# jack-nie/bitcoin-miner

Hardware: AMD Instinct MI355X
Metric: GH/s (SHA-256 nonce search) at 1/2/4/8 MI355X; % of VALU int roofline (higher is better)
Workload: dtype u32

## Files before the change

### bitcoin-miner_amd/csrc/minehip.cpp

```cpp
#include <hip/hip_runtime.h>
#include <stdio.h>
#include <stdlib.h>
#include <string.h>

#include <algorithm>
#include <atomic>
#include <chrono>
#include <cmath>
#include <condition_variable>
#include <memory>
#include <mutex>
#include <string>
#include <system_error>
#include <thread>
#include <vector>

#include "../../include/minehip.h"
#include "../../include/minehip_server.h"
#include "layout.hpp"
#include "msgcodec.hpp"
#include "multi.hpp"
#include "plan.hpp"
#include "sched.hpp"

namespace mh {
hipError_t fast_module_init(int dev);
#ifdef MH_DEV_HOOKS
hipError_t fast_keep_ok(int dev, bool* ok);
hipError_t set_hash_xor(int dev, uint64_t x, hipStream_t s, bool* fast_ok);
#endif
hipError_t launch_fast(int dev, int J, int mode, const FastArgs& a, Partial* partials, hipStream_t s);
hipError_t launch_generic_scan(const GenArgs& a, Partial* partials, uint32_t blocks, hipStream_t s);
hipError_t launch_hash_batch(const GenArgs& a, const uint64_t* d_nonces, uint64_t* d_out, uint64_t n,
                             hipStream_t s);
hipError_t launch_merge(const Partial* partials, uint32_t n, Partial* best, hipStream_t s);
hipError_t launch_fast_first(int dev, int J, int mode, const FastArgs& a, Partial* partials, const FirstArgs& f,
                             bool stop, hipStream_t s);
hipError_t launch_generic_scan_first(const GenArgs& a, Partial* partials, uint32_t blocks, const FirstArgs& f,
                                     hipStream_t s);
hipError_t launch_finish_first(const GenArgs& a, const Partial* best, const unsigned long long* scanned, uint64_t* out,
                               hipStream_t s);
hipError_t launch_fast_hits(int dev, int J, int mode, const FastArgs& a, Partial* partials, const HitsArgs& h,
                            hipStream_t s);
hipError_t launch_generic_scan_hits(const GenArgs& a, Partial* partials, uint32_t blocks, const HitsArgs& h,
                                    hipStream_t s);
hipError_t launch_fast_hits_stop(int dev, int J, int mode, const FastArgs& a, Partial* partials, const HitsStopArgs& h,
                                 hipStream_t s);
hipError_t launch_generic_scan_hits_stop(const GenArgs& a, Partial* partials, uint32_t blocks, const HitsStopArgs& h,
                                         hipStream_t s);
hipError_t launch_batch_scan(const BatchEntry* entries, const uint32_t* tile_entry, Partial* partials, uint32_t tiles,
                             hipStream_t s);
hipError_t launch_merge_segments(const Partial* partials, const uint32_t* seg, Partial* results, uint32_t requests,
                                 hipStream_t s);
hipError_t launch_batch_scan_slots(const BatchEntry* entries, const uint32_t* tile_entry, Partial* partials,
                                   uint32_t tiles, hipStream_t s);
hipError_t launch_batch_fast(int dev, int J, int mode, const BatchFastItem* items, const uint32_t* chunk_item,
                             Partial* partials, uint32_t chunks, hipStream_t s);
#ifdef MH_DEV_HOOKS
hipError_t batch_fast_hooks(int dev, uint64_t x, hipStream_t s, bool* keep_ok, bool* xor_ok);
#endif
hipError_t launch_batch_scan_first(const BatchEntry* entries, const uint32_t* tile_entry, const uint32_t* entry_req,
                                   const uint32_t* order, BatchFirstWords* words, Partial* partials, uint32_t tiles,
                                   hipStream_t s);
hipError_t launch_merge_segments_first(const Partial* partials, const uint32_t* seg, const BatchEntry* entries,
                                       const uint32_t* tile_entry, const BatchFirstWords* words,
                                       BatchFirstResult* results, uint32_t requests, hipStream_t s);
hipError_t launch_batch_scan_first_slots(const BatchEntry* entries, const uint32_t* tile_entry,
                                         const uint32_t* entry_req, const uint32_t* order, BatchFirstWords* words,
                                         Partial* partials, uint32_t tiles, hipStream_t s);
hipError_t launch_merge_segments_first_ex(const Partial* partials, const uint32_t* seg, const GenArgs* req_gen,
                                          const BatchFirstWords* words, BatchFirstResult* results, uint32_t requests,
                                          hipStream_t s);
hipError_t launch_batch_first(int dev, int J, int mode, const BatchFirstItem* items, const uint32_t* chunk_item,
                              const uint32_t* order, Partial* partials, uint32_t chunks, hipStream_t s);
hipError_t launch_batch_stop(int dev, int J, int mode, const BatchFirstItem* items, const uint32_t* chunk_item,
                             const uint32_t* order, Partial* partials, uint32_t chunks, hipStream_t s);
hipError_t launch_batch_scan_hits(const BatchEntry* entries, const uint32_t* tile_entry, const uint32_t* entry_req,
                                  BatchHitsWords* words, Hit* hits, Partial* partials, uint32_t tiles,
                                  hipStream_t s);
hipError_t launch_batch_scan_hits_slots(const BatchEntry* entries, const uint32_t* tile_entry, const uint32_t* entry_req,
                                        BatchHitsWords* words, Hit* hits, Partial* partials, uint32_t tiles,
                                        hipStream_t s);
hipError_t launch_batch_hits(int dev, int J, int mode, const BatchHitsItem* items, const uint32_t* chunk_item,
                             Partial* partials, uint32_t chunks, hipStream_t s);
hipError_t launch_batch_scan_bound(bool slots, const BatchEntry* entries, const uint32_t* tile_entry,
                                   const uint32_t* entry_req, const uint32_t* order, BatchBoundWords* words,
                                   uint32_t* slices, Hit* hits, Partial* partials, uint32_t tiles, hipStream_t s);
hipError_t launch_batch_bound(int dev, int J, int mode, const BatchBoundItem* items, const uint32_t* chunk_item,
                              const uint32_t* order, Partial* partials, uint32_t chunks, hipStream_t s);
hipError_t launch_merge_segments_bound(const Partial* partials, const uint32_t* seg, const BatchBoundWords* words,
                                       const Hit* hits, Hit* packed, uint64_t limit, const unsigned long long* base_in,
                                       unsigned long long* base_out, BatchBoundResult* results, uint32_t requests,
                                       hipStream_t s);
hipError_t launch_merge_segments_hits(const Partial* partials, const uint32_t* seg, const BatchHitsWords* words,
                                      const Hit* hits, Hit* packed, uint64_t limit, const unsigned long long* base_in,
                                      unsigned long long* base_out, BatchHitsResult* results, uint32_t requests,
                                      hipStream_t s);
}

namespace {

using mh::Partial;

thread_local std::string g_err;

int fail(int code, const std::string& what) {
    g_err = what;
    return code;
}

}

namespace mh {
int set_error(int code, const char* what) { return fail(code, what); }
}

namespace {

#define MH_HIP(call)                                                                                 \
    do {                                                                                             \
        hipError_t e_ = (call);                                                                      \
        if (e_ != hipSuccess) return fail(MH_EHIP, std::string(#call) + ": " + hipGetErrorString(e_)); \
    } while (0)

constexpr uint64_t kBatchChunk = 1u << 22;
constexpr int kEventPairs = 512;
constexpr uint32_t kQueueSlots = 4096;
constexpr size_t kBatchTableBytes = 4u << 20;
constexpr uint32_t kBatchResults = 1u << 16;
constexpr size_t kFirstBatchFastTableBytes = 5u << 20;
static_assert(8u * (size_t)mh::kMaxBlocksPerLaunch + mh::kBatchMaxEntries * (sizeof(mh::BatchEntry) + 4u) +
                      (mh::kBatchMaxRequests + 1u) * 4u +
                      mh::kBatchMaxRequests * (sizeof(mh::GenArgs) + sizeof(mh::BatchFirstWords)) +
                      mh::kBatchMaxFastItems * sizeof(mh::BatchFirstItem) + 9u * 16u <= kFirstBatchFastTableBytes,
              "a first-hit pass with fast pieces fits its table buffer");
static_assert(8u * (size_t)mh::kMaxBlocksPerLaunch + mh::kBatchMaxEntries * (sizeof(mh::BatchEntry) + 4u) +
                      (mh::kBatchMaxRequests + 1u) * 4u + mh::kBatchMaxRequests * sizeof(mh::BatchBoundWords) +
                      mh::kBatchMaxFastItems * sizeof(mh::BatchBoundItem) + 9u * 16u <= kFirstBatchFastTableBytes,
              "a first-k-hits pass fits its table buffer");

struct Timed {
    hipEvent_t start = nullptr, stop = nullptr;
    int kind;
    int var;
};

struct VarStat {
    uint64_t launches = 0, nonces = 0, ns = 0, ops = 0, slots = 0;
};
constexpr int kVariants = 16 * mh::kModes * 5;
inline int var_index(int J, int mode, int L) { return J + 16 * mode + 16 * mh::kModes * (L - 1); }

struct DevCtx {
    std::mutex mu;
    int dev = -1;
    bool ready = false;
    hipStream_t stream = nullptr;
    hipStream_t ps[2] = {nullptr, nullptr};
    hipEvent_t ev_piece[2] = {nullptr, nullptr};
    hipEvent_t ev_main = nullptr;
    Partial* d_partials = nullptr;
    Partial* d_best = nullptr;
    Partial* h_best = nullptr;
    uint64_t* d_nonces = nullptr;
    uint64_t* d_hashes = nullptr;
    uint32_t poff = 0;
    uint32_t* d_counters = nullptr;
    uint32_t qoff = 0;
    uint8_t* d_btab = nullptr;
    uint8_t* h_btab = nullptr;
    Partial* d_bres = nullptr;
    Partial* h_bres = nullptr;
    mh::BatchFirstResult* d_fres = nullptr;
    mh::BatchFirstResult* h_fres = nullptr;
    uint8_t* d_ftab = nullptr;
    uint8_t* h_ftab = nullptr;
    uint64_t* d_first = nullptr;
    uint64_t* h_first = nullptr;
    const mh::FirstArgs* first = nullptr;
    bool first_stop = false;
    mh::Hit* d_hits = nullptr;
    uint64_t* d_hcursor = nullptr;
    uint64_t* h_hcursor = nullptr;
    const mh::HitsArgs* hits = nullptr;
    uint64_t* d_fhits = nullptr;
    uint32_t* d_slices = nullptr;
    uint64_t* h_fhits = nullptr;
    const mh::HitsStopArgs* hits_stop = nullptr;
    mh::BatchHitsResult* d_hres = nullptr;
    mh::BatchHitsResult* h_hres = nullptr;
    mh::Hit* d_hpacked = nullptr;
    uint64_t* d_hbase = nullptr;
    mh::BatchBoundResult* d_kres = nullptr;
    mh::BatchBoundResult* h_kres = nullptr;
    uint32_t* d_bslices = nullptr;
#ifdef MH_DEV_HOOKS
    uint32_t keep = 0;
    bool keep_fast = false;
    bool xor_on = false;
    bool xor_fast = false;
#endif
    bool prof = false;
    std::vector<Timed> pool;
    int used = 0;
    uint64_t cnt[8] = {0};
    VarStat var[kVariants];
};

std::mutex g_tab_mu;
std::vector<std::unique_ptr<DevCtx>> g_tab;
int g_ndev = -1;

int device_count_impl() {
    std::lock_guard<std::mutex> lk(g_tab_mu);
    if (g_ndev < 0) {
        int n = 0;
        if (hipGetDeviceCount(&n) != hipSuccess) n = 0;
        g_ndev = n;
        g_tab.resize((size_t)n);
        for (auto& p : g_tab) p.reset(new DevCtx());
    }
    return g_ndev;
}

int get_ctx(int dev, DevCtx** out) {
    const int n = device_count_impl();
    if (n <= 0) return fail(MH_ENODEV, "no HIP device visible");
    if (dev < 0 || dev >= n) return fail(MH_EINVAL, "device index out of range");
    DevCtx* c = g_tab[(size_t)dev].get();
    *out = c;
    return MH_OK;
}

int init_locked(DevCtx* c, int dev) {
    if (c->ready) return MH_OK;
    MH_HIP(hipSetDevice(dev));
    hipDeviceProp_t prop;
    MH_HIP(hipGetDeviceProperties(&prop, dev));
    if (strncmp(prop.gcnArchName, "gfx950", 6) != 0)
        return fail(MH_ENODEV, std::string("device is ") + prop.gcnArchName + ", kernels are built for gfx950 only");
    if (!c->stream) MH_HIP(hipStreamCreateWithFlags(&c->stream, hipStreamNonBlocking));
    if (!c->ps[0] || !c->ps[1]) {
        int least = 0, greatest = 0;
        MH_HIP(hipDeviceGetStreamPriorityRange(&least, &greatest));
        if (!c->ps[0]) MH_HIP(hipStreamCreateWithPriority(&c->ps[0], hipStreamNonBlocking, greatest));
        if (!c->ps[1]) MH_HIP(hipStreamCreateWithPriority(&c->ps[1], hipStreamNonBlocking, least));
    }
    for (auto& e : c->ev_piece)
        if (!e) MH_HIP(hipEventCreateWithFlags(&e, hipEventDisableTiming));
    if (!c->ev_main) MH_HIP(hipEventCreateWithFlags(&c->ev_main, hipEventDisableTiming));
    if (!c->d_partials) MH_HIP(hipMalloc(&c->d_partials, sizeof(Partial) * mh::kMaxBlocksPerLaunch));
    if (!c->d_best) MH_HIP(hipMalloc(&c->d_best, sizeof(Partial)));
    if (!c->d_counters) MH_HIP(hipMalloc(&c->d_counters, sizeof(uint32_t) * kQueueSlots));
    if (!c->h_best) MH_HIP(hipHostMalloc(&c->h_best, sizeof(Partial), hipHostMallocDefault));
    if (!c->d_nonces) MH_HIP(hipMalloc(&c->d_nonces, sizeof(uint64_t) * kBatchChunk));
    if (!c->d_hashes) MH_HIP(hipMalloc(&c->d_hashes, sizeof(uint64_t) * kBatchChunk));
    if (c->pool.empty()) c->pool.resize(kEventPairs);
    for (auto& t : c->pool) {
        if (!t.start) MH_HIP(hipEventCreate(&t.start));
        if (!t.stop) MH_HIP(hipEventCreate(&t.stop));
    }
    MH_HIP(mh::fast_module_init(dev));
    c->dev = dev;
    c->ready = true;
    return MH_OK;
}

#ifdef MH_DEV_HOOKS
int read_hash_keep(DevCtx* c) {
    c->keep = 0;
    c->keep_fast = false;
    const char* e = getenv("MINEHIP_DEV_HASH_KEEP");
    if (!e || !*e) return MH_OK;
    unsigned k0 = 0, k1 = 0;
    char rest = 0;
    if (sscanf(e, "%u,%u%c", &k0, &k1, &rest) != 2 || k0 > 32u || k1 > 32u)
        return fail(MH_EINVAL, "MINEHIP_DEV_HASH_KEEP: expected k0,k1 with 0 <= k <= 32");
    MH_HIP(mh::fast_keep_ok(c->dev, &c->keep_fast));
    c->keep = mh::keep_word(k0, k1);
    return MH_OK;
}

int read_hash_xor(DevCtx* c) {
    c->xor_on = c->xor_fast = false;
    const char* e = getenv("MINEHIP_DEV_HASH_XOR");
    uint64_t x = 0;
    if (e && *e) {
        size_t n = 0;
        for (; e[n]; ++n) {
            const char ch = e[n];
            const int v = (ch >= '0' && ch <= '9') ? ch - '0' : (ch >= 'a' && ch <= 'f') ? ch - 'a' + 10
                        : (ch >= 'A' && ch <= 'F') ? ch - 'A' + 10 : -1;
            if (v < 0 || n >= 16) return fail(MH_EINVAL, "MINEHIP_DEV_HASH_XOR: expected 1 to 16 hex digits");
            x = (x << 4) | (uint64_t)v;
        }
    }
    MH_HIP(mh::set_hash_xor(c->dev, x, c->stream, &c->xor_fast));
    c->xor_on = x != 0;
    return MH_OK;
}
#endif

int harvest_locked(DevCtx* c) {
    for (int i = 0; i < c->used; ++i) {
        float ms = 0.f;
        MH_HIP(hipEventElapsedTime(&ms, c->pool[(size_t)i].start, c->pool[(size_t)i].stop));
        const uint64_t ns = (uint64_t)((double)ms * 1.0e6);
        c->cnt[c->pool[(size_t)i].kind == 0 ? 2 : 5] += ns;
        if (c->pool[(size_t)i].kind == 0) c->var[c->pool[(size_t)i].var].ns += ns;
    }
    c->used = 0;
    return MH_OK;
}

int piece_streams_wait_main(DevCtx* c) {
    MH_HIP(hipEventRecord(c->ev_main, c->stream));
    for (auto s : c->ps) MH_HIP(hipStreamWaitEvent(s, c->ev_main, 0));
    return MH_OK;
}

int flush_partials(DevCtx* c, bool split) {
    if (!c->poff) return MH_OK;
    if (split) {
        for (int k = 0; k < 2; ++k) {
            MH_HIP(hipEventRecord(c->ev_piece[k], c->ps[k]));
            MH_HIP(hipStreamWaitEvent(c->stream, c->ev_piece[k], 0));
        }
    }
    MH_HIP(mh::launch_merge(c->d_partials, c->poff, c->d_best, c->stream));
    c->poff = 0;
    if (split) return piece_streams_wait_main(c);
    return MH_OK;
}

bool coarse_piece(const mh::Piece& p, const mh::PlanOpts& opt) { return p.kind == 0 && p.L == opt.lower_digits; }

bool early_piece_ok(const mh::FastArgs& a, int word) {
    const uint32_t J = (uint32_t)word;
    if ((a.inner >> 2) != J || a.hole + a.hole_w > a.n_hi + a.L) return false;
    for (uint32_t j = 0; j + 1u < a.L; ++j) {
        const uint32_t pos = a.g_last - j - (j >= a.g_hole ? 1u : 0u);
        if (pos > a.g_last || (pos >> 2) != J) return false;
    }
    return true;
}

int enqueue_piece(DevCtx* c, const mh::Piece& p, const mh::PlanOpts& opt, bool split) {
    hipStream_t s = !split ? c->stream : c->ps[coarse_piece(p, opt) ? 0 : 1];
    uint32_t blocks;
    if (p.kind == 0) {
        if (p.fa.n_runs == 0 || p.fa.L < 1 || p.fa.L > 5 || p.fa.n_hi + p.fa.L > 20)
            return fail(MH_EINTERNAL, "internal: bad fast piece");
        if (p.fa.mode >= mh::kModeOneEarly && !early_piece_ok(p.fa, p.J))
            return fail(MH_EINTERNAL, "internal: bad Early piece (an enumerated digit outside word J)");
        blocks = (p.fa.n_runs + mh::kBlockThreads - 1) / mh::kBlockThreads;
    } else {
        if (p.ga.count == 0 || p.ga.count > (uint64_t)mh::kMaxBlocksPerLaunch * mh::kBlockThreads)
            return fail(MH_EINTERNAL, "internal: bad generic piece");
        blocks = (uint32_t)((p.ga.count + mh::kBlockThreads - 1) / mh::kBlockThreads);
    }
    if (blocks > mh::kMaxBlocksPerLaunch) return fail(MH_EINTERNAL, "internal: grid too large");
    if (c->poff + blocks > mh::kMaxBlocksPerLaunch) {
        const int rc = flush_partials(c, split);
        if (rc) return rc;
    }
    Partial* out = c->d_partials + c->poff;
    Timed* tm = nullptr;
    mh::FastArgs fa = p.fa;
#ifdef MH_DEV_HOOKS
    mh::GenArgs ga = p.ga;
    ga.pad = c->keep;
    if (p.kind == 0) {
        if (c->keep && !c->keep_fast)
            return fail(MH_EINVAL, "MINEHIP_DEV_HASH_KEEP is set but the fast code object is not the coarse-hash "
                                   "variant (MINEHIP_DEV_CODE_OBJECT=build/fast_search_keep.hsaco)");
        if (c->xor_on && !c->xor_fast)
            return fail(MH_EINVAL, "MINEHIP_DEV_HASH_XOR is set but the fast code object has no mh_dev_hash_xor "
                                   "(MINEHIP_DEV_CODE_OBJECT=build/fast_search_keep.hsaco)");
        fa.pad_ = c->keep;
    }
#else
    const mh::GenArgs& ga = p.ga;
#endif
    if (p.kind == 0) {
        fa.n_chunks = blocks;
        fa.counter = (opt.queue && c->qoff < kQueueSlots) ? c->d_counters + c->qoff++ : nullptr;
    }
    if (c->prof) {
        if (c->used == kEventPairs) {
            MH_HIP(hipStreamSynchronize(c->stream));
            for (auto ps : c->ps) MH_HIP(hipStreamSynchronize(ps));
            int rc = harvest_locked(c);
            if (rc) return rc;
        }
        tm = &c->pool[(size_t)c->used++];
        tm->kind = p.kind;
        tm->var = p.kind == 0 ? var_index(p.J, p.mode, p.L) : 0;
        MH_HIP(hipEventRecord(tm->start, s));
    }
    if (c->first) {
        if (p.kind == 0)
            MH_HIP(mh::launch_fast_first(c->dev, p.J, p.mode, fa, out, *c->first, c->first_stop, s));
        else
            MH_HIP(mh::launch_generic_scan_first(ga, out, blocks, *c->first, s));
    } else if (c->hits_stop) {
        if (p.kind == 0)
            MH_HIP(mh::launch_fast_hits_stop(c->dev, p.J, p.mode, fa, out, *c->hits_stop, s));
        else
            MH_HIP(mh::launch_generic_scan_hits_stop(ga, out, blocks, *c->hits_stop, s));
    } else if (c->hits) {
        if (p.kind == 0)
            MH_HIP(mh::launch_fast_hits(c->dev, p.J, p.mode, fa, out, *c->hits, s));
        else
            MH_HIP(mh::launch_generic_scan_hits(ga, out, blocks, *c->hits, s));
    } else if (p.kind == 0)
        MH_HIP(mh::launch_fast(c->dev, p.J, p.mode, fa, out, s));
    else
        MH_HIP(mh::launch_generic_scan(ga, out, blocks, s));
    if (tm) MH_HIP(hipEventRecord(tm->stop, s));
    c->poff += blocks;
    if (c->prof) {
        if (p.kind == 0) {
            const uint64_t n = p.count;
            c->cnt[0] += 1;
            c->cnt[1] += n;
            c->cnt[3] += n * (uint64_t)p.ops;
            c->cnt[6] += n * (uint64_t)p.slots;
            VarStat& v = c->var[var_index(p.J, p.mode, p.L)];
            v.launches += 1;
            v.nonces += n;
            v.ops += n * (uint64_t)p.ops;
            v.slots += n * (uint64_t)p.slots;
        } else {
            c->cnt[4] += p.count;
        }
    }
    return MH_OK;
}

mh::PlanOpts plan_opts() {
    mh::PlanOpts o;
    if (const char* e = getenv("MINEHIP_LOWER_DIGITS")) {
        const int v = atoi(e);
        if (v >= 1 && v <= 5) o.lower_digits = v;
    }
    if (const char* e = getenv("MINEHIP_MIN_LANES")) o.min_lanes = strtoull(e, nullptr, 10);
    if (const char* e = getenv("MINEHIP_LAUNCH_NONCES")) {
        const unsigned long long v = strtoull(e, nullptr, 10);
        if (v >= 1) o.max_nonces_per_launch = v;
    }
    if (const char* e = getenv("MINEHIP_GENERIC_BELOW")) o.generic_below = strtoull(e, nullptr, 10);
    if (const char* e = getenv("MINEHIP_MAX_BLOCKS")) {
        const unsigned long long v = strtoull(e, nullptr, 10);
        if (v >= 1 && v <= mh::kMaxBlocksPerLaunch) o.max_blocks = (uint32_t)v;
    }
    if (const char* e = getenv("MINEHIP_STREAMS")) {
        const int v = atoi(e);
        if (v == 1 || v == 2) o.streams = v;
    }
    if (const char* e = getenv("MINEHIP_FINE_TAIL")) o.fine_tail = strtoull(e, nullptr, 10);
    if (const char* e = getenv("MINEHIP_QUEUE")) {
        const int v = atoi(e);
        if (v == 0 || v == 1) o.queue = v;
    }
    if (const char* e = getenv("MINEHIP_EARLY")) {
        const int v = atoi(e);
        if (v == 0 || v == 1) o.early = v;
    }
    return o;
}

uint64_t now_ns() {
    return (uint64_t)std::chrono::duration_cast<std::chrono::nanoseconds>(
               std::chrono::steady_clock::now().time_since_epoch())
        .count();
}

int search_impl(int dev, const mh::Prefix& pre, uint64_t lower, uint64_t upper, uint64_t* oh, uint64_t* on,
                uint64_t* busy_ns = nullptr) {
    DevCtx* c;
    int rc = get_ctx(dev, &c);
    if (rc) return rc;
    std::lock_guard<std::mutex> lk(c->mu);
    rc = init_locked(c, dev);
    if (rc) return rc;
    const uint64_t t0 = now_ns();
    MH_HIP(hipSetDevice(dev));
#ifdef MH_DEV_HOOKS
    rc = read_hash_keep(c);
    if (rc) return rc;
    rc = read_hash_xor(c);
    if (rc) return rc;
#endif
    MH_HIP(hipMemsetAsync(c->d_best, 0xFF, sizeof(Partial), c->stream));
    const mh::PlanOpts opt = plan_opts();
    if (opt.queue) MH_HIP(hipMemsetAsync(c->d_counters, 0, sizeof(uint32_t) * kQueueSlots, c->stream));
    c->qoff = 0;
    bool any_coarse = false, any_fine = false;
    if (opt.streams == 2)
        mh::plan_search(pre, lower, upper, opt, [&](const mh::Piece& p) {
            (coarse_piece(p, opt) ? any_coarse : any_fine) = true;
            return !(any_coarse && any_fine);
        });
    const bool split = opt.streams == 2 && any_coarse && any_fine;
    if (split) {
        rc = piece_streams_wait_main(c);
        if (rc) return rc;
    }
    int err = MH_OK;
    c->poff = 0;
    mh::plan_search(pre, lower, upper, opt, [&](const mh::Piece& p) {
        err = enqueue_piece(c, p, opt, split);
        return err == MH_OK;
    });
    if (!err) err = flush_partials(c, split);
    if (err) {
        for (auto ps : c->ps)
            if (ps) (void)hipStreamSynchronize(ps);
        (void)hipStreamSynchronize(c->stream);
        return err;
    }
    MH_HIP(hipMemcpyAsync(c->h_best, c->d_best, sizeof(Partial), hipMemcpyDeviceToHost, c->stream));
    MH_HIP(hipStreamSynchronize(c->stream));
    if (c->prof) {
        rc = harvest_locked(c);
        if (rc) return rc;
    }
    *oh = c->h_best->hash;
    *on = c->h_best->nonce;
    if (busy_ns) *busy_ns = now_ns() - t0;
    return MH_OK;
}

int search_first_impl(int dev, const mh::Prefix& pre, uint64_t lower, uint64_t upper, uint64_t target, uint32_t flags,
                      mh_first* out) {
    DevCtx* c;
    int rc = get_ctx(dev, &c);
    if (rc) return rc;
    std::lock_guard<std::mutex> lk(c->mu);
    rc = init_locked(c, dev);
    if (rc) return rc;
    MH_HIP(hipSetDevice(dev));
    if (!c->d_first) MH_HIP(hipMalloc(&c->d_first, 5 * sizeof(uint64_t)));
    if (!c->h_first) MH_HIP(hipHostMalloc(&c->h_first, 3 * sizeof(uint64_t), hipHostMallocDefault));
#ifdef MH_DEV_HOOKS
    c->keep = 0;
    c->keep_fast = c->xor_on = c->xor_fast = false;
#endif
    MH_HIP(hipMemsetAsync(c->d_best, 0xFF, sizeof(Partial), c->stream));
    MH_HIP(hipMemsetAsync(c->d_first, 0xFF, sizeof(uint64_t), c->stream));
    MH_HIP(hipMemsetAsync(c->d_first + 1, 0, sizeof(uint64_t), c->stream));
    const mh::PlanOpts opt = plan_opts();
    if (opt.queue) MH_HIP(hipMemsetAsync(c->d_counters, 0, sizeof(uint32_t) * kQueueSlots, c->stream));
    c->qoff = 0;
    bool any_coarse = false, any_fine = false;
    if (opt.streams == 2)
        mh::plan_search(pre, lower, upper, opt, [&](const mh::Piece& p) {
            (coarse_piece(p, opt) ? any_coarse : any_fine) = true;
            return !(any_coarse && any_fine);
        });
    const bool split = opt.streams == 2 && any_coarse && any_fine;
    if (split) {
        rc = piece_streams_wait_main(c);
        if (rc) return rc;
    }
    const mh::FirstArgs fargs{target, (unsigned long long*)c->d_first, (unsigned long long*)(c->d_first + 1)};
    int err = MH_OK;
    c->poff = 0;
    c->first = &fargs;
    c->first_stop = (flags & MH_FIRST_STOP_RUNNING) != 0;
    mh::plan_search(pre, lower, upper, opt, [&](const mh::Piece& p) {
        err = enqueue_piece(c, p, opt, split);
        return err == MH_OK;
    });
    c->first = nullptr;
    c->first_stop = false;
    if (!err) err = flush_partials(c, split);
    if (err) {
        for (auto ps : c->ps)
            if (ps) (void)hipStreamSynchronize(ps);
        (void)hipStreamSynchronize(c->stream);
        return err;
    }
    mh::GenArgs ga;
    mh::make_gen_args(pre, &ga);
    MH_HIP(mh::launch_finish_first(ga, c->d_best, (const unsigned long long*)(c->d_first + 1), c->d_first + 2, c->stream));
    MH_HIP(hipMemcpyAsync(c->h_first, c->d_first + 2, 3 * sizeof(uint64_t), hipMemcpyDeviceToHost, c->stream));
    MH_HIP(hipStreamSynchronize(c->stream));
    if (c->prof) {
        rc = harvest_locked(c);
        if (rc) return rc;
    }
    out->hash = c->h_first[0];
    out->nonce = c->h_first[1];
    out->scanned = c->h_first[2];
    out->found = out->hash <= target ? 1 : 0;
    out->reserved = 0;
    return MH_OK;
}

uint64_t hits_slots() {
    if (const char* e = getenv("MINEHIP_HITS_SLOTS")) {
        const unsigned long long v = strtoull(e, nullptr, 10);
        if (v >= 1 && v <= MH_HITS_MAX_CAP) return v;
    }
    return MH_HITS_MAX_CAP;
}

int hits_scan_range(DevCtx* c, const mh::Prefix& pre, uint64_t lower, uint64_t upper, uint64_t target, uint64_t slots,
                    uint64_t* count, std::vector<mh::Hit>* got) {
    MH_HIP(hipMemsetAsync(c->d_best, 0xFF, sizeof(Partial), c->stream));
    MH_HIP(hipMemsetAsync(c->d_hcursor, 0, sizeof(uint64_t), c->stream));
    const mh::PlanOpts opt = plan_opts();
    if (opt.queue) MH_HIP(hipMemsetAsync(c->d_counters, 0, sizeof(uint32_t) * kQueueSlots, c->stream));
    c->qoff = 0;
    bool any_coarse = false, any_fine = false;
    if (opt.streams == 2)
        mh::plan_search(pre, lower, upper, opt, [&](const mh::Piece& p) {
            (coarse_piece(p, opt) ? any_coarse : any_fine) = true;
            return !(any_coarse && any_fine);
        });
    const bool split = opt.streams == 2 && any_coarse && any_fine;
    if (split) {
        const int rc = piece_streams_wait_main(c);
        if (rc) return rc;
    }
    const mh::HitsArgs hargs{target, (unsigned long long*)c->d_hcursor, c->d_hits, slots};
    int err = MH_OK;
    c->poff = 0;
    c->hits = &hargs;
    mh::plan_search(pre, lower, upper, opt, [&](const mh::Piece& p) {
        err = enqueue_piece(c, p, opt, split);
        return err == MH_OK;
    });
    c->hits = nullptr;
    if (!err) err = flush_partials(c, split);
    if (err) {
        for (auto ps : c->ps)
            if (ps) (void)hipStreamSynchronize(ps);
        (void)hipStreamSynchronize(c->stream);
        return err;
    }
    MH_HIP(hipMemcpyAsync(c->h_best, c->d_best, sizeof(Partial), hipMemcpyDeviceToHost, c->stream));
    MH_HIP(hipMemcpyAsync(c->h_hcursor, c->d_hcursor, sizeof(uint64_t), hipMemcpyDeviceToHost, c->stream));
    MH_HIP(hipStreamSynchronize(c->stream));
    if (c->prof) {
        const int rc = harvest_locked(c);
        if (rc) return rc;
    }
    *count = *c->h_hcursor;
    if (got) {
        got->resize((size_t)std::min(*count, slots));
        if (!got->empty()) MH_HIP(hipMemcpy(got->data(), c->d_hits, got->size() * sizeof(mh::Hit), hipMemcpyDeviceToHost));
    }
    return MH_OK;
}

bool hit_by_nonce(const mh::Hit& x, const mh::Hit& y) { return x.nonce < y.nonce; }

int hits_window_walk(DevCtx* c, const mh::Prefix& pre, uint64_t lower, uint64_t upper, uint64_t target, uint64_t slots,
                     uint64_t want, double spacing, std::vector<mh::Hit>* list, bool widen = false) {
    const double per_window = std::max(1.0, (double)slots / 4.0 * spacing);
    uint64_t w = per_window >= 9.0e18 ? (uint64_t)9.0e18 : (uint64_t)per_window;
    const uint64_t w0 = w;
    std::vector<mh::Hit> win;
    uint64_t cur = lower;
    list->clear();
    while (list->size() < want) {
        const uint64_t hi = (upper - cur < w - 1u) ? upper : cur + (w - 1u);
        uint64_t wc = 0;
        const int rc = hits_scan_range(c, pre, cur, hi, target, slots, &wc, &win);
        if (rc) return rc;
        if (wc > slots) {
            w = (hi - cur + 1u) / 2u;
            continue;
        }
        std::sort(win.begin(), win.end(), hit_by_nonce);
        list->insert(list->end(), win.begin(), win.end());
        if (hi == upper) break;
        cur = hi + 1u;
        if (widen && w < w0) w = w0 - w < w ? w0 : w * 2u;
    }
    return MH_OK;
}

int search_hits_impl(int dev, const mh::Prefix& pre, uint64_t lower, uint64_t upper, uint64_t target, mh_hit* hits,
                     size_t cap, mh_hits* out) {
    DevCtx* c;
    int rc = get_ctx(dev, &c);
    if (rc) return rc;
    std::lock_guard<std::mutex> lk(c->mu);
    rc = init_locked(c, dev);
    if (rc) return rc;
    MH_HIP(hipSetDevice(dev));
    if (!c->d_hits) MH_HIP(hipMalloc(&c->d_hits, sizeof(mh::Hit) * MH_HITS_MAX_CAP));
    if (!c->d_hcursor) MH_HIP(hipMalloc(&c->d_hcursor, sizeof(uint64_t)));
    if (!c->h_hcursor) MH_HIP(hipHostMalloc(&c->h_hcursor, sizeof(uint64_t), hipHostMallocDefault));
#ifdef MH_DEV_HOOKS
    c->keep = 0;
    c->keep_fast = c->xor_on = c->xor_fast = false;
#endif
    const uint64_t slots = hits_slots();
    std::vector<mh::Hit> got;
    uint64_t count = 0;
    rc = hits_scan_range(c, pre, lower, upper, target, slots, &count, cap ? &got : nullptr);
    if (rc) return rc;
    out->count = count;
    out->stored = std::min<uint64_t>(count, cap);
    out->hash = c->h_best->hash;
    out->nonce = c->h_best->nonce;
    if (cap && count > slots) {
        const double total = (double)(upper - lower) + 1.0;
        std::vector<mh::Hit> list;
        rc = hits_window_walk(c, pre, lower, upper, target, slots, out->stored, total / (double)count, &list);
        if (rc) return rc;
        if (list.size() < out->stored) return fail(MH_EINTERNAL, "internal: the hit windows hold fewer hits than the scan counted");
        got.swap(list);
    } else {
        std::sort(got.begin(), got.end(), hit_by_nonce);
    }
    for (uint64_t i = 0; i < out->stored; ++i) hits[i] = mh_hit{got[(size_t)i].hash, got[(size_t)i].nonce};
    return MH_OK;
}

int search_first_hits_impl(int dev, const mh::Prefix& pre, uint64_t lower, uint64_t upper, uint64_t target, mh_hit* hits,
                           size_t k, mh_first_hits* out, bool widen_walk = false) {
    DevCtx* c;
    int rc = get_ctx(dev, &c);
    if (rc) return rc;
    std::lock_guard<std::mutex> lk(c->mu);
    rc = init_locked(c, dev);
    if (rc) return rc;
    MH_HIP(hipSetDevice(dev));
    if (!c->d_hits) MH_HIP(hipMalloc(&c->d_hits, sizeof(mh::Hit) * MH_HITS_MAX_CAP));
    if (!c->d_hcursor) MH_HIP(hipMalloc(&c->d_hcursor, sizeof(uint64_t)));
    if (!c->h_hcursor) MH_HIP(hipHostMalloc(&c->h_hcursor, sizeof(uint64_t), hipHostMallocDefault));
    if (!c->d_fhits) MH_HIP(hipMalloc(&c->d_fhits, 2 * sizeof(uint64_t)));
    if (!c->d_slices) MH_HIP(hipMalloc(&c->d_slices, sizeof(uint32_t) * mh::kFirstHitsSlices));
    if (!c->h_fhits) MH_HIP(hipHostMalloc(&c->h_fhits, sizeof(uint64_t), hipHostMallocDefault));
#ifdef MH_DEV_HOOKS
    c->keep = 0;
    c->keep_fast = c->xor_on = c->xor_fast = false;
#endif
    const uint64_t slots = hits_slots();
    const uint64_t total_m1 = upper - lower;
    MH_HIP(hipMemsetAsync(c->d_best, 0xFF, sizeof(Partial), c->stream));
    MH_HIP(hipMemsetAsync(c->d_hcursor, 0, sizeof(uint64_t), c->stream));
    MH_HIP(hipMemsetAsync(c->d_fhits, 0xFF, sizeof(uint64_t), c->stream));
    MH_HIP(hipMemsetAsync(c->d_fhits + 1, 0, sizeof(uint64_t), c->stream));
    MH_HIP(hipMemsetAsync(c->d_slices, 0, sizeof(uint32_t) * mh::kFirstHitsSlices, c->stream));
    const mh::PlanOpts opt = plan_opts();
    if (opt.queue) MH_HIP(hipMemsetAsync(c->d_counters, 0, sizeof(uint32_t) * kQueueSlots, c->stream));
    c->qoff = 0;
    bool any_coarse = false, any_fine = false;
    if (opt.streams == 2)
        mh::plan_search(pre, lower, upper, opt, [&](const mh::Piece& p) {
            (coarse_piece(p, opt) ? any_coarse : any_fine) = true;
            return !(any_coarse && any_fine);
        });
    const bool split = opt.streams == 2 && any_coarse && any_fine;
    if (split) {
        rc = piece_streams_wait_main(c);
        if (rc) return rc;
    }
    const mh::HitsStopArgs hs{mh::HitsArgs{target, (unsigned long long*)c->d_hcursor, c->d_hits, slots},
                              (uint64_t)k,
                              (unsigned long long*)c->d_fhits,
                              c->d_slices,
                              lower,
                              total_m1,
                              mh::first_hits_shift(total_m1),
                              0u,
                              (unsigned long long*)(c->d_fhits + 1)};
    int err = MH_OK;
    c->poff = 0;
    c->hits_stop = &hs;
    mh::plan_search(pre, lower, upper, opt, [&](const mh::Piece& p) {
        err = enqueue_piece(c, p, opt, split);
        return err == MH_OK;
    });
    c->hits_stop = nullptr;
    if (!err) err = flush_partials(c, split);
    if (err) {
        for (auto ps : c->ps)
            if (ps) (void)hipStreamSynchronize(ps);
        (void)hipStreamSynchronize(c->stream);
        return err;
    }
    MH_HIP(hipMemcpyAsync(c->h_best, c->d_best, sizeof(Partial), hipMemcpyDeviceToHost, c->stream));
    MH_HIP(hipMemcpyAsync(c->h_hcursor, c->d_hcursor, sizeof(uint64_t), hipMemcpyDeviceToHost, c->stream));
    MH_HIP(hipMemcpyAsync(c->h_fhits, c->d_fhits + 1, sizeof(uint64_t), hipMemcpyDeviceToHost, c->stream));
    MH_HIP(hipStreamSynchronize(c->stream));
    if (c->prof) {
        rc = harvest_locked(c);
        if (rc) return rc;
    }
    const uint64_t appended = *c->h_hcursor, scanned = *c->h_fhits;
    const Partial best = *c->h_best;
    std::vector<mh::Hit> got;
    if (appended <= slots) {
        got.resize((size_t)appended);
        if (!got.empty()) MH_HIP(hipMemcpy(got.data(), c->d_hits, got.size() * sizeof(mh::Hit), hipMemcpyDeviceToHost));
        std::sort(got.begin(), got.end(), hit_by_nonce);
    } else {
        rc = hits_window_walk(c, pre, lower, upper, target, slots, k, std::max(1.0, (double)scanned) / (double)appended, &got,
                              widen_walk);
        if (rc) return rc;
    }
    out->stored = std::min<uint64_t>(got.size(), k);
    out->scanned = scanned;
    if (out->stored < k) {
        if (scanned != total_m1 + 1u)
            return fail(MH_EINTERNAL, "internal: fewer than k hits, but the scan did not hash the whole range");
        out->hash = best.hash;
        out->nonce = best.nonce;
    } else {
        out->hash = got[0].hash;
        out->nonce = got[0].nonce;
        for (size_t i = 1; i < k; ++i)
            if (got[i].hash < out->hash || (got[i].hash == out->hash && got[i].nonce < out->nonce)) {
                out->hash = got[i].hash;
                out->nonce = got[i].nonce;
            }
    }
    for (uint64_t i = 0; i < out->stored; ++i) hits[i] = mh_hit{got[(size_t)i].hash, got[(size_t)i].nonce};
    return MH_OK;
}

int check_common(const uint8_t* msg, size_t len) {
    if (msg == nullptr && len != 0) return fail(MH_EINVAL, "msg is NULL");
    if (len > MH_MAX_MSG_LEN) return fail(MH_ETOOLONG, "message longer than MH_MAX_MSG_LEN");
    return MH_OK;
}


uint32_t batch_slots() {
    if (const char* e = getenv("MINEHIP_BATCH_SLOTS")) {
        const unsigned long long v = strtoull(e, nullptr, 10);
        if (v >= 1 && v <= mh::kMaxBlocksPerLaunch) return (uint32_t)v;
    }
    return mh::kMaxBlocksPerLaunch;
}

inline size_t align16(size_t x) { return (x + 15u) & ~(size_t)15u; }

int batch_init_locked(DevCtx* c) {
    if (!c->d_btab) MH_HIP(hipMalloc(&c->d_btab, kBatchTableBytes));
    if (!c->h_btab) MH_HIP(hipHostMalloc(&c->h_btab, kBatchTableBytes, hipHostMallocDefault));
    if (!c->d_bres) MH_HIP(hipMalloc(&c->d_bres, sizeof(Partial) * kBatchResults));
    if (!c->h_bres) MH_HIP(hipHostMalloc(&c->h_bres, sizeof(Partial) * kBatchResults, hipHostMallocDefault));
    return MH_OK;
}

struct BatchPending {
    std::vector<size_t> req_idx;
    size_t toff = 0;
};

int batch_drain(DevCtx* c, const mh::BatchRequest* reqs, BatchPending* pend, mh_result* out) {
    MH_HIP(hipStreamSynchronize(c->stream));
    if (c->prof) {
        const int rc = harvest_locked(c);
        if (rc) return rc;
    }
    for (size_t k = 0; k < pend->req_idx.size(); ++k) {
        mh_result& r = out[reqs[pend->req_idx[k]].id];
        r.hash = c->h_bres[k].hash;
        r.nonce = c->h_bres[k].nonce;
    }
    pend->req_idx.clear();
    pend->toff = 0;
    return MH_OK;
}

int batch_run_pass(DevCtx* c, const mh::BatchRequest* reqs, const mh::BatchTables& t, uint32_t slot_cap,
                   BatchPending* pend, mh_result* out) {
    if (!mh::batch_tables_ok(t, slot_cap)) return fail(MH_EINTERNAL, "internal: bad batch tables");
    const size_t ne = t.entries.size(), nreq = t.req_idx.size(), tiles = t.tile_entry.size();
    const size_t o_seg = align16(ne * sizeof(mh::BatchEntry)), o_tile = o_seg + align16((nreq + 1u) * sizeof(uint32_t));
    const size_t bytes = o_tile + align16(tiles * sizeof(uint32_t));
    if (bytes > kBatchTableBytes || nreq > kBatchResults) return fail(MH_EINTERNAL, "internal: batch pass too large");
    if (pend->toff + bytes > kBatchTableBytes || pend->req_idx.size() + nreq > kBatchResults ||
        (c->prof && c->used == kEventPairs)) {
        const int rc = batch_drain(c, reqs, pend, out);
        if (rc) return rc;
    }
    uint8_t* h = c->h_btab + pend->toff;
    uint8_t* d = c->d_btab + pend->toff;
    memcpy(h, t.entries.data(), ne * sizeof(mh::BatchEntry));
#ifdef MH_DEV_HOOKS
    for (size_t i = 0; i < ne; ++i) ((mh::BatchEntry*)h)[i].g.pad = c->keep;
#endif
    memcpy(h + o_seg, t.seg.data(), (nreq + 1u) * sizeof(uint32_t));
    memcpy(h + o_tile, t.tile_entry.data(), tiles * sizeof(uint32_t));
    MH_HIP(hipMemcpyAsync(d, h, bytes, hipMemcpyHostToDevice, c->stream));
    Timed* tm = nullptr;
    if (c->prof) {
        tm = &c->pool[(size_t)c->used++];
        tm->kind = 1;
        tm->var = 0;
        MH_HIP(hipEventRecord(tm->start, c->stream));
    }
    MH_HIP(mh::launch_batch_scan((const mh::BatchEntry*)d, (const uint32_t*)(d + o_tile), c->d_partials, (uint32_t)tiles,
                                 c->stream));
    if (tm) {
        MH_HIP(hipEventRecord(tm->stop, c->stream));
        c->cnt[4] += t.nonces;
    }
    const size_t roff = pend->req_idx.size();
    MH_HIP(mh::launch_merge_segments(c->d_partials, (const uint32_t*)(d + o_seg), c->d_bres + roff, (uint32_t)nreq,
                                     c->stream));
    MH_HIP(hipMemcpyAsync(c->h_bres + roff, c->d_bres + roff, nreq * sizeof(Partial), hipMemcpyDeviceToHost, c->stream));
    pend->req_idx.insert(pend->req_idx.end(), t.req_idx.begin(), t.req_idx.end());
    pend->toff += bytes;
    return MH_OK;
}

int batch_run_fused(int dev, const mh::BatchRequest* reqs, const std::vector<mh::BatchItem>& items, int passes,
                    uint32_t slot_cap, mh_result* out) {
    DevCtx* c;
    int rc = get_ctx(dev, &c);
    if (rc) return rc;
    std::lock_guard<std::mutex> lk(c->mu);
    rc = init_locked(c, dev);
    if (rc) return rc;
    MH_HIP(hipSetDevice(dev));
    rc = batch_init_locked(c);
    if (rc) return rc;
#ifdef MH_DEV_HOOKS
// ... 2064 lines not shown
```

### bitcoin-miner_amd/csrc/search_kernels.hip

```cpp
#include <hip/hip_runtime.h>

#include <algorithm>
#include <stdio.h>
#include <stdlib.h>

#include <map>
#include <mutex>
#include <string>
#include <utility>

#include "kernel_common.hpp"
#include "layout.hpp"
#include "sha256_gfx950.hpp"

extern "C" const unsigned char mh_fast_co_begin[];
extern "C" const unsigned char mh_first_co_begin[];
extern "C" const unsigned char mh_hits_co_begin[];
extern "C" const unsigned char mh_batch_co_begin[];
extern "C" const unsigned char mh_batch_first_co_begin[];
extern "C" const unsigned char mh_first_stop_co_begin[];
extern "C" const unsigned char mh_batch_first_stop_co_begin[];
extern "C" const unsigned char mh_batch_hits_co_begin[];
extern "C" const unsigned char mh_hits_stop_co_begin[];
extern "C" const unsigned char mh_batch_bound_co_begin[];
// ... 119 lines not shown
            ((uint64_t)(uint32_t)__builtin_amdgcn_readlane((int)(uint32_t)(taken >> 32), (int)lead) << 32) |
            (uint32_t)__builtin_amdgcn_readlane((int)(uint32_t)taken, (int)lead);
        const uint64_t slot = base + (uint32_t)__builtin_popcountll(hm & ((1ull << lane) - 1ull));
        if (hit && slot < h.cap) h.hits[slot] = Hit{hash, nonce};
    }
    if (gid >= a.count) {
        hash = ~0ull;
        nonce = ~0ull;
    }
    block_min(hash, nonce);
    if (threadIdx.x == 0) partials[blockIdx.x] = Partial{hash, nonce};
}

__global__ __launch_bounds__(kBlockThreads) void generic_scan_hits_stop(const GenArgs a, Partial* __restrict__ partials,
                                                                        const HitsStopArgs hs) {
    using namespace dev;
    __shared__ uint32_t s_skip;
    const uint64_t base = a.first + (uint64_t)blockIdx.x * kBlockThreads;
    if (threadIdx.x == 0)
        s_skip = base > __hip_atomic_load(hs.bound, __ATOMIC_RELAXED, __HIP_MEMORY_SCOPE_AGENT) ? 1u : 0u;
    __syncthreads();
    if (s_skip) {
        if (threadIdx.x == 0) partials[blockIdx.x] = Partial{~0ull, ~0ull};
        return;
    }
    const uint64_t n = base + threadIdx.x;
    const uint64_t left = a.count - (uint64_t)blockIdx.x * kBlockThreads;
    uint32_t h0, h1;
    hash_generic(a, n, h0, h1);
    uint64_t hash = ((uint64_t)h0 << 32) | h1, nonce = n;
    const bool hit = threadIdx.x < left && hash <= hs.h.target;
    const uint64_t hm = __builtin_amdgcn_ballot_w64(hit);
    if (hm) {
        const uint32_t lane = __builtin_amdgcn_mbcnt_hi(~0u, __builtin_amdgcn_mbcnt_lo(~0u, 0u));
        const uint32_t lead = (uint32_t)__builtin_ctzll(hm);
        uint32_t back = 0u;
        if (hit) back = atomicAdd(first_hits_slice(hs, n), 1u);
        asm volatile("" ::"v"(back) : "memory");
        unsigned long long taken = 0ull;
        if (lane == lead) taken = atomicAdd(hs.h.cursor, (unsigned long long)__builtin_popcountll(hm));
        const uint64_t first =
            ((uint64_t)(uint32_t)__builtin_amdgcn_readlane((int)(uint32_t)(taken >> 32), (int)lead) << 32) |
            (uint32_t)__builtin_amdgcn_readlane((int)(uint32_t)taken, (int)lead);
        const uint64_t slot = first + (uint32_t)__builtin_popcountll(hm & ((1ull << lane) - 1ull));
        if (hit && slot < hs.h.cap) hs.h.hits[slot] = Hit{hash, nonce};
        if (first + (uint32_t)__builtin_popcountll(hm) >= hs.k) publish_first_hits_bound(hs, lane);
    }
    if (threadIdx.x >= left) {
        hash = ~0ull;
        nonce = ~0ull;
    }
    block_min(hash, nonce);
    if (threadIdx.x == 0) {
        partials[blockIdx.x] = Partial{hash, nonce};
        atomicAdd(hs.scanned, (unsigned long long)(left < (uint64_t)kBlockThreads ? left : (uint64_t)kBlockThreads));
    }
}

__global__ void finish_first(const GenArgs a, const Partial* __restrict__ best,
                             const unsigned long long* __restrict__ scanned, uint64_t* __restrict__ out) {
    Partial b = *best;
    if (b.hash == 0ull) {
        uint32_t h0, h1;
        dev::hash_generic(a, b.nonce, h0, h1);
        b.hash = ((uint64_t)h0 << 32) | h1;
    }
    out[0] = b.hash;
    out[1] = b.nonce;
    out[2] = *scanned;
}

__global__ __launch_bounds__(kBlockThreads) void hash_batch(const GenArgs a, const uint64_t* __restrict__ nonces,
                                                            uint64_t* __restrict__ out, uint64_t n) {
    const uint64_t i = (uint64_t)blockIdx.x * kBlockThreads + threadIdx.x;
    if (i >= n) return;
    uint32_t h0, h1;
    dev::hash_generic(a, nonces[i], h0, h1);
    out[i] = ((uint64_t)h0 << 32) | h1;
}

constexpr int kMergeThreads = 1024;
constexpr int kMergeUnroll = 8;

__global__ __launch_bounds__(kMergeThreads) void merge_partials(const Partial* __restrict__ p, uint32_t n,
                                                                Partial* __restrict__ best) {
    using namespace dev;
    uint64_t h = ~0ull, nn = ~0ull;
    for (uint32_t base = 0; base < n; base += kMergeThreads * kMergeUnroll) {
        Partial x[kMergeUnroll];
#pragma unroll
        for (int u = 0; u < kMergeUnroll; ++u) {
            const uint32_t i = base + (uint32_t)u * kMergeThreads + threadIdx.x;
            x[u] = (i < n) ? p[i] : Partial{~0ull, ~0ull};
        }
#pragma unroll
        for (int u = 0; u < kMergeUnroll; ++u)
            if (lex_less(x[u].hash, x[u].nonce, h, nn)) {
                h = x[u].hash;
                nn = x[u].nonce;
            }
    }
    block_min<kMergeThreads>(h, nn);
    if (threadIdx.x == 0) {
        const Partial b = *best;
        if (lex_less(h, nn, b.hash, b.nonce)) *best = Partial{h, nn};
    }
}

namespace dev {

template <bool FIRST, bool HITS = false, bool BOUND = false>
__device__ __forceinline__ void scan_decade(const GenArgs& a, uint64_t u, uint32_t jlo, uint32_t jhi, uint64_t target,
                                            uint64_t& bh, uint64_t& bn, unsigned long long* cursor = nullptr,
                                            Hit* region = nullptr, uint64_t region_slots = 0,
                                            const HitsStopArgs* hs = nullptr, bool live = true) {
    constexpr uint64_t P10[19] = {1ull, 10ull, 100ull, 1000ull, 10000ull, 100000ull, 1000000ull, 10000000ull,
                                  100000000ull, 1000000000ull, 10000000000ull, 100000000000ull, 1000000000000ull,
                                  10000000000000ull, 100000000000000ull, 1000000000000000ull, 10000000000000000ull,
                                  100000000000000000ull, 1000000000000000000ull};
    uint32_t nu = 0;
#pragma unroll
    for (int k = 0; k < 19; ++k) nu += (u >= P10[k]) ? 1u : 0u;
    uint32_t w[32];
#pragma unroll
    for (int x = 0; x < 16; ++x) w[x] = a.tail[x];
#pragma unroll
    for (int x = 16; x < 32; ++x) w[x] = 0u;
    uint64_t q = u;
#pragma unroll
    for (int k = 0; k < 19; ++k) {
        if ((uint32_t)k < nu) {
            const uint64_t q10 = q / 10u;
            const uint32_t dg = (uint32_t)(q - q10 * 10u);
            q = q10;
            const uint32_t pos = a.t + nu - 1u - (uint32_t)k;
            add_word(w, pos >> 2, (0x30u + dg) << (24u - 8u * (pos & 3u)));
        }
    }
    const uint32_t last = a.t + nu;
    const uint32_t lsh = 24u - 8u * (last & 3u);
    add_word(w, last >> 2, 0x30u << lsh);
    const uint32_t end = last + 1u;
    add_word(w, end >> 2, 0x80u << (24u - 8u * (end & 3u)));
    const uint64_t bits = (a.plen + nu + 1u) * 8u;
    const bool two = end + 9u > 64u;
    const uint32_t bhi = (uint32_t)(bits >> 32), blo = (uint32_t)bits;
    w[14] = two ? w[14] : bhi;
    w[15] = two ? w[15] : blo;
    w[30] = two ? bhi : 0u;
    w[31] = two ? blo : 0u;
    const bool in1 = last >= 64u;
    const bool both = two && !in1;
    const uint32_t jw = (last >> 2) & 15u;
    uint32_t st[8];
#pragma unroll
    for (int i = 0; i < 8; ++i) st[i] = a.mid[i];
    if (in1) sha256_block(st, w);
    uint32_t v[16];
#pragma unroll
    for (int x = 0; x < 16; ++x) {
        const uint32_t lo = w[x], hi = w[16 + x];
        v[x] = in1 ? hi : lo;
    }
    const uint32_t w16 = w[16];
    const uint64_t n0 = u * 10u;
#pragma unroll 1
    for (uint32_t j = BOUND ? 0u : jlo; j <= (BOUND ? 9u : jhi); ++j) {
        const uint32_t dj = j << lsh;
        uint32_t x[16];
#pragma unroll
        for (int i = 0; i < 16; ++i) x[i] = v[i] | ((jw == (uint32_t)i) ? dj : 0u);
        uint32_t s[8];
#pragma unroll
        for (int i = 0; i < 8; ++i) s[i] = st[i];
        if (both) {
            sha256_block(s, x);
#pragma unroll
            for (int i = 0; i < 16; ++i) x[i] = 0u;
            x[0] = w16;
            x[14] = bhi;
            x[15] = blo;
        }
        uint32_t h0, h1;
        sha256_block_h01(s, x, h0, h1);
#ifdef MH_DEV_HOOKS
        if constexpr (!FIRST && !HITS) {
            h0 = (h0 ^ mh_dev_hash_xor[0]) & keep_mask0(a.pad);
            h1 = (h1 ^ mh_dev_hash_xor[1]) & keep_mask1(a.pad);
// ... 818 lines not shown
hipError_t launch_batch_scan_first(const BatchEntry* entries, const uint32_t* tile_entry, const uint32_t* entry_req,
                                   const uint32_t* order, BatchFirstWords* words, Partial* partials, uint32_t tiles,
                                   hipStream_t s) {
    hipLaunchKernelGGL(batch_scan_first, dim3(tiles), dim3(kBlockThreads), 0, s, entries, tile_entry, entry_req, order,
                       words, partials);
    return hipGetLastError();
}

hipError_t launch_merge_segments_first(const Partial* partials, const uint32_t* seg, const BatchEntry* entries,
                                       const uint32_t* tile_entry, const BatchFirstWords* words,
                                       BatchFirstResult* results, uint32_t requests, hipStream_t s) {
    hipLaunchKernelGGL(merge_segments_first, dim3(requests), dim3(kBlockThreads), 0, s, partials, seg, entries,
                       tile_entry, words, results);
    return hipGetLastError();
}

hipError_t launch_batch_scan_first_slots(const BatchEntry* entries, const uint32_t* tile_entry,
                                         const uint32_t* entry_req, const uint32_t* order, BatchFirstWords* words,
                                         Partial* partials, uint32_t tiles, hipStream_t s) {
    hipLaunchKernelGGL(batch_scan_first_slots, dim3(tiles), dim3(kBlockThreads), 0, s, entries, tile_entry, entry_req,
                       order, words, partials);
    return hipGetLastError();
}

hipError_t launch_merge_segments_first_ex(const Partial* partials, const uint32_t* seg, const GenArgs* req_gen,
                                          const BatchFirstWords* words, BatchFirstResult* results, uint32_t requests,
                                          hipStream_t s) {
    hipLaunchKernelGGL(merge_segments_first_ex, dim3(requests), dim3(kBlockThreads), 0, s, partials, seg, req_gen, words,
                       results);
    return hipGetLastError();
}

hipError_t launch_batch_scan_hits(const BatchEntry* entries, const uint32_t* tile_entry, const uint32_t* entry_req,
                                  BatchHitsWords* words, Hit* hits, Partial* partials, uint32_t tiles,
                                  hipStream_t s) {
    hipLaunchKernelGGL(batch_scan_hits, dim3(tiles), dim3(kBlockThreads), 0, s, entries, tile_entry, entry_req, words,
                       hits, partials);
    return hipGetLastError();
}

hipError_t launch_batch_scan_hits_slots(const BatchEntry* entries, const uint32_t* tile_entry, const uint32_t* entry_req,
                                        BatchHitsWords* words, Hit* hits, Partial* partials, uint32_t tiles,
                                        hipStream_t s) {
    hipLaunchKernelGGL(batch_scan_hits_slots, dim3(tiles), dim3(kBlockThreads), 0, s, entries, tile_entry, entry_req,
                       words, hits, partials);
    return hipGetLastError();
}

hipError_t launch_merge_segments_hits(const Partial* partials, const uint32_t* seg, const BatchHitsWords* words,
                                      const Hit* hits, Hit* packed, uint64_t limit, const unsigned long long* base_in,
                                      unsigned long long* base_out, BatchHitsResult* results, uint32_t requests,
                                      hipStream_t s) {
    hipLaunchKernelGGL(merge_segments_hits, dim3(requests), dim3(kBlockThreads), 0, s, partials, seg, words, hits, packed,
                       limit, base_in, base_out, results);
    return hipGetLastError();
}

hipError_t launch_batch_scan_bound(bool slots, const BatchEntry* entries, const uint32_t* tile_entry,
                                   const uint32_t* entry_req, const uint32_t* order, BatchBoundWords* words,
                                   uint32_t* slices, Hit* hits, Partial* partials, uint32_t tiles, hipStream_t s) {
    if (slots)
        hipLaunchKernelGGL(batch_scan_bound_slots, dim3(tiles), dim3(kBlockThreads), 0, s, entries, tile_entry, entry_req,
                           order, words, slices, hits, partials);
    else
        hipLaunchKernelGGL(batch_scan_bound, dim3(tiles), dim3(kBlockThreads), 0, s, entries, tile_entry, entry_req, order,
                           words, slices, hits, partials);
    return hipGetLastError();
}

hipError_t launch_merge_segments_bound(const Partial* partials, const uint32_t* seg, const BatchBoundWords* words,
                                       const Hit* hits, Hit* packed, uint64_t limit, const unsigned long long* base_in,
                                       unsigned long long* base_out, BatchBoundResult* results, uint32_t requests,
                                       hipStream_t s) {
    hipLaunchKernelGGL(merge_segments_bound, dim3(requests), dim3(kBlockThreads), 0, s, partials, seg, words, hits, packed,
                       limit, base_in, base_out, results);
    return hipGetLastError();
}

hipError_t launch_merge(const Partial* partials, uint32_t n, Partial* best, hipStream_t s) {
    hipLaunchKernelGGL(merge_partials, dim3(1), dim3(kMergeThreads), 0, s, partials, n, best);
    return hipGetLastError();
}

}
```

Measured before the change: 54.10.

## Fuse final merge with result writeback and state reset; stream pieces without pre-plan pass

```diff
diff --git a/bitcoin-miner_amd/csrc/minehip.cpp b/bitcoin-miner_amd/csrc/minehip.cpp
--- a/bitcoin-miner_amd/csrc/minehip.cpp
+++ b/bitcoin-miner_amd/csrc/minehip.cpp
@@ -2,6 +2,7 @@
 #include <stdio.h>
 #include <stdlib.h>
 #include <string.h>
+#include <unistd.h>
 
 #include <algorithm>
 #include <atomic>
@@ -34,6 +35,8 @@
 hipError_t launch_hash_batch(const GenArgs& a, const uint64_t* d_nonces, uint64_t* d_out, uint64_t n,
                              hipStream_t s);
 hipError_t launch_merge(const Partial* partials, uint32_t n, Partial* best, hipStream_t s);
+hipError_t launch_merge_final(const Partial* partials, uint32_t n, Partial* best, Partial* result, uint32_t* counters,
+                              uint32_t n_counters, hipStream_t s);
 hipError_t launch_fast_first(int dev, int J, int mode, const FastArgs& a, Partial* partials, const FirstArgs& f,
                              bool stop, hipStream_t s);
 hipError_t launch_generic_scan_first(const GenArgs& a, Partial* partials, uint32_t blocks, const FirstArgs& f,
@@ -162,11 +165,17 @@
     Partial* d_partials = nullptr;
     Partial* d_best = nullptr;
     Partial* h_best = nullptr;
+    Partial* h_best_dev = nullptr;
+    bool dirty = true;
     uint64_t* d_nonces = nullptr;
     uint64_t* d_hashes = nullptr;
     uint32_t poff = 0;
     uint32_t* d_counters = nullptr;
     uint32_t qoff = 0;
+    mh::PlanOpts opt;
+    std::string opt_env;
+    bool opt_valid = false;
+    std::vector<mh::Piece> ahead;
     uint8_t* d_btab = nullptr;
     uint8_t* h_btab = nullptr;
     Partial* d_bres = nullptr;
@@ -252,7 +261,8 @@
     if (!c->d_partials) MH_HIP(hipMalloc(&c->d_partials, sizeof(Partial) * mh::kMaxBlocksPerLaunch));
     if (!c->d_best) MH_HIP(hipMalloc(&c->d_best, sizeof(Partial)));
     if (!c->d_counters) MH_HIP(hipMalloc(&c->d_counters, sizeof(uint32_t) * kQueueSlots));
-    if (!c->h_best) MH_HIP(hipHostMalloc(&c->h_best, sizeof(Partial), hipHostMallocDefault));
+    if (!c->h_best) MH_HIP(hipHostMalloc(&c->h_best, sizeof(Partial), hipHostMallocMapped | hipHostMallocCoherent));
+    if (!c->h_best_dev) MH_HIP(hipHostGetDevicePointer((void**)&c->h_best_dev, c->h_best, 0));
     if (!c->d_nonces) MH_HIP(hipMalloc(&c->d_nonces, sizeof(uint64_t) * kBatchChunk));
     if (!c->d_hashes) MH_HIP(hipMalloc(&c->d_hashes, sizeof(uint64_t) * kBatchChunk));
     if (c->pool.empty()) c->pool.resize(kEventPairs);
@@ -330,6 +340,18 @@
     MH_HIP(mh::launch_merge(c->d_partials, c->poff, c->d_best, c->stream));
     c->poff = 0;
     if (split) return piece_streams_wait_main(c);
+    return MH_OK;
+}
+
+int finish_search(DevCtx* c, bool split) {
+    if (split) {
+        for (int k = 0; k < 2; ++k) {
+            MH_HIP(hipEventRecord(c->ev_piece[k], c->ps[k]));
+            MH_HIP(hipStreamWaitEvent(c->stream, c->ev_piece[k], 0));
+        }
+    }
+    MH_HIP(mh::launch_merge_final(c->d_partials, c->poff, c->d_best, c->h_best_dev, c->d_counters, c->qoff, c->stream));
+    c->poff = 0;
     return MH_OK;
 }
 
@@ -470,6 +492,22 @@
     return o;
 }
 
+const mh::PlanOpts& search_opts(DevCtx* c) {
+    thread_local std::string now;
+    now.clear();
+    for (char** e = environ; e && *e; ++e)
+        if (strncmp(*e, "MINEHIP_", 8) == 0) {
+            now += *e;
+            now += '\n';
+        }
+    if (!c->opt_valid || now != c->opt_env) {
+        c->opt = plan_opts();
+        c->opt_env = now;
+        c->opt_valid = true;
+    }
+    return c->opt;
+}
+
 uint64_t now_ns() {
     return (uint64_t)std::chrono::duration_cast<std::chrono::nanoseconds>(
                std::chrono::steady_clock::now().time_since_epoch())
@@ -492,36 +530,53 @@
     rc = read_hash_xor(c);
     if (rc) return rc;
 #endif
-    MH_HIP(hipMemsetAsync(c->d_best, 0xFF, sizeof(Partial), c->stream));
-    const mh::PlanOpts opt = plan_opts();
-    if (opt.queue) MH_HIP(hipMemsetAsync(c->d_counters, 0, sizeof(uint32_t) * kQueueSlots, c->stream));
+    const bool reset = c->dirty;
+    c->dirty = true;
+    if (reset) {
+        MH_HIP(hipMemsetAsync(c->d_best, 0xFF, sizeof(Partial), c->stream));
+        MH_HIP(hipMemsetAsync(c->d_counters, 0, sizeof(uint32_t) * kQueueSlots, c->stream));
+    }
+    const mh::PlanOpts& opt = search_opts(c);
     c->qoff = 0;
-    bool any_coarse = false, any_fine = false;
-    if (opt.streams == 2)
-        mh::plan_search(pre, lower, upper, opt, [&](const mh::Piece& p) {
-            (coarse_piece(p, opt) ? any_coarse : any_fine) = true;
-            return !(any_coarse && any_fine);
-        });
-    const bool split = opt.streams == 2 && any_coarse && any_fine;
-    if (split) {
-        rc = piece_streams_wait_main(c);
-        if (rc) return rc;
-    }
+    c->poff = 0;
+    constexpr size_t kAhead = 32;
+    bool any_coarse = false, any_fine = false, decided = opt.streams != 2, split = false;
     int err = MH_OK;
-    c->poff = 0;
+    c->ahead.clear();
+    auto start = [&]() {
+        decided = true;
+        split = opt.streams == 2 && any_coarse && any_fine;
+        if (split && reset) err = piece_streams_wait_main(c);
+        for (size_t i = 0; i < c->ahead.size() && !err; ++i) err = enqueue_piece(c, c->ahead[i], opt, split);
+        c->ahead.clear();
+    };
     mh::plan_search(pre, lower, upper, opt, [&](const mh::Piece& p) {
-        err = enqueue_piece(c, p, opt, split);
+        if (decided) {
+            err = enqueue_piece(c, p, opt, split);
+            return err == MH_OK;
+        }
+        (coarse_piece(p, opt) ? any_coarse : any_fine) = true;
+        c->ahead.push_back(p);
+        if (!(any_coarse && any_fine)) {
+            if (c->ahead.size() < kAhead) return true;
+            mh::plan_search(pre, lower, upper, opt, [&](const mh::Piece& q) {
+                (coarse_piece(q, opt) ? any_coarse : any_fine) = true;
+                return !(any_coarse && any_fine);
+            });
+        }
+        start();
         return err == MH_OK;
     });
-    if (!err) err = flush_partials(c, split);
+    if (!decided) start();
+    if (!err) err = finish_search(c, split);
     if (err) {
         for (auto ps : c->ps)
             if (ps) (void)hipStreamSynchronize(ps);
         (void)hipStreamSynchronize(c->stream);
         return err;
     }
-    MH_HIP(hipMemcpyAsync(c->h_best, c->d_best, sizeof(Partial), hipMemcpyDeviceToHost, c->stream));
     MH_HIP(hipStreamSynchronize(c->stream));
+    c->dirty = false;
     if (c->prof) {
         rc = harvest_locked(c);
         if (rc) return rc;
@@ -547,6 +602,7 @@
     c->keep = 0;
     c->keep_fast = c->xor_on = c->xor_fast = false;
 #endif
+    c->dirty = true;
     MH_HIP(hipMemsetAsync(c->d_best, 0xFF, sizeof(Partial), c->stream));
     MH_HIP(hipMemsetAsync(c->d_first, 0xFF, sizeof(uint64_t), c->stream));
     MH_HIP(hipMemsetAsync(c->d_first + 1, 0, sizeof(uint64_t), c->stream));
@@ -609,6 +665,7 @@
 
 int hits_scan_range(DevCtx* c, const mh::Prefix& pre, uint64_t lower, uint64_t upper, uint64_t target, uint64_t slots,
                     uint64_t* count, std::vector<mh::Hit>* got) {
+    c->dirty = true;
     MH_HIP(hipMemsetAsync(c->d_best, 0xFF, sizeof(Partial), c->stream));
     MH_HIP(hipMemsetAsync(c->d_hcursor, 0, sizeof(uint64_t), c->stream));
     const mh::PlanOpts opt = plan_opts();
@@ -744,6 +801,7 @@
 #endif
     const uint64_t slots = hits_slots();
     const uint64_t total_m1 = upper - lower;
+    c->dirty = true;
     MH_HIP(hipMemsetAsync(c->d_best, 0xFF, sizeof(Partial), c->stream));
     MH_HIP(hipMemsetAsync(c->d_hcursor, 0, sizeof(uint64_t), c->stream));
     MH_HIP(hipMemsetAsync(c->d_fhits, 0xFF, sizeof(uint64_t), c->stream));
@@ -845,6 +903,7 @@
 inline size_t align16(size_t x) { return (x + 15u) & ~(size_t)15u; }
 
 int batch_init_locked(DevCtx* c) {
+    c->dirty = true;
     if (!c->d_btab) MH_HIP(hipMalloc(&c->d_btab, kBatchTableBytes));
     if (!c->h_btab) MH_HIP(hipHostMalloc(&c->h_btab, kBatchTableBytes, hipHostMallocDefault));
     if (!c->d_bres) MH_HIP(hipMalloc(&c->d_bres, sizeof(Partial) * kBatchResults));
diff --git a/bitcoin-miner_amd/csrc/search_kernels.hip b/bitcoin-miner_amd/csrc/search_kernels.hip
--- a/bitcoin-miner_amd/csrc/search_kernels.hip
+++ b/bitcoin-miner_amd/csrc/search_kernels.hip
@@ -225,10 +225,10 @@
 constexpr int kMergeThreads = 1024;
 constexpr int kMergeUnroll = 8;
 
-__global__ __launch_bounds__(kMergeThreads) void merge_partials(const Partial* __restrict__ p, uint32_t n,
-                                                                Partial* __restrict__ best) {
-    using namespace dev;
-    uint64_t h = ~0ull, nn = ~0ull;
+namespace dev {
+
+__device__ __forceinline__ void fold_partials(const Partial* __restrict__ p, uint32_t n, uint64_t& h, uint64_t& nn) {
+    h = nn = ~0ull;
     for (uint32_t base = 0; base < n; base += kMergeThreads * kMergeUnroll) {
         Partial x[kMergeUnroll];
 #pragma unroll
@@ -244,9 +244,39 @@
             }
     }
     block_min<kMergeThreads>(h, nn);
+}
+
+}
+
+__global__ __launch_bounds__(kMergeThreads) void merge_partials(const Partial* __restrict__ p, uint32_t n,
+                                                                Partial* __restrict__ best) {
+    using namespace dev;
+    uint64_t h, nn;
+    fold_partials(p, n, h, nn);
     if (threadIdx.x == 0) {
         const Partial b = *best;
         if (lex_less(h, nn, b.hash, b.nonce)) *best = Partial{h, nn};
+    }
+}
+
+__global__ __launch_bounds__(kMergeThreads) void merge_partials_final(const Partial* __restrict__ p, uint32_t n,
+                                                                      Partial* __restrict__ best,
+                                                                      Partial* __restrict__ result,
+                                                                      uint32_t* __restrict__ counters,
+                                                                      uint32_t n_counters) {
+    using namespace dev;
+    uint64_t h, nn;
+    fold_partials(p, n, h, nn);
+    for (uint32_t i = threadIdx.x; i < n_counters; i += kMergeThreads) counters[i] = 0u;
+    if (threadIdx.x == 0) {
+        const Partial b = *best;
+        if (lex_less(b.hash, b.nonce, h, nn)) {
+            h = b.hash;
+            nn = b.nonce;
+        }
+        *result = Partial{h, nn};
+        __threadfence_system();
+        *best = Partial{~0ull, ~0ull};
     }
 }
 
@@ -1231,4 +1261,11 @@
     return hipGetLastError();
 }
 
-}
+hipError_t launch_merge_final(const Partial* partials, uint32_t n, Partial* best, Partial* result, uint32_t* counters,
+                              uint32_t n_counters, hipStream_t s) {
+    hipLaunchKernelGGL(merge_partials_final, dim3(1), dim3(kMergeThreads), 0, s, partials, n, best, result, counters,
+                       n_counters);
+    return hipGetLastError();
+}
+
+}
```

Result: no change. 54.31, median of 4 (+0.4%).
